# Youngju-Na/UFORecon

Hardware: AMD Instinct MI355X
Metric: rays/s (per-ray volume-rendering path, 64+64 hierarchical samples, DTU-shaped 3-view 512x640) (higher is better)
Workload: dtype f32; 1 GPU; configs[1]: full 512x640 frame = 327680 rays, 3 source views, 64+64 samples, rays sharded by row tiles over 1 GPU(s), depth/RGB tiles all-gathered; rays_per_frame=327680, chunk_rays=4096, side_streams=3

## Files before the change

uforecon_amd/csrc/api_weights_frame.hip:

```cpp
#include "api_common.h"
#include "ufr_layout_f16.h"

using namespace ufr;
using namespace ufr::api;

namespace {

int frame_check(const ufr_frame_desc* d) {
  UFR_REQUIRE(d, "frame desc is null");
  UFR_CHECK(check_views("frame desc", d->NV));
  UFR_REQUIRE(d->H >= 8 && d->W >= 8 && d->H % 4 == 0 && d->W % 4 == 0, "H,W must be multiples of 4 (got %dx%d)",
              d->H, d->W);
  UFR_REQUIRE(d->source_imgs && d->depth_info && d->feat, "null frame tensor");
  UFR_REQUIRE((long long)d->H * d->W < (1 << 24) && (long long)(d->H / 4) * (d->W / 4) * 32 * (d->NV - 1) < (1ll << 32),
              "image of %dx%d is too large for the gather's 24-bit texel indices", d->H, d->W);
  {
    const long long px = (long long)d->H * d->W, mpx = (long long)(d->H / 4) * (d->W / 4), lim = 1ll << 31;
    UFR_REQUIRE(px * 16 < lim && d->NV * mpx * 128 < lim && d->NV * mpx * 32 * (d->NV - 1) * 4 < lim,
                "frame of %dx%d with %d views: an image / feature-map buffer reaches 2 GiB (the gathers' zero-fill offset)",
                d->H, d->W, d->NV);
  }
  const bool has_vol = d->vol_feat[0] != nullptr;
  for (int s = 0; s < UFR_NUM_STAGES; ++s) {
    UFR_REQUIRE((d->vol_feat[s] != nullptr) == has_vol && (d->vol_weight[s] != nullptr) == has_vol,
                "volumes must be given for all stages or for none (stage %d)", s + 1);
    if (has_vol) UFR_REQUIRE(d->vol_D[s] >= 2 && d->vol_H[s] >= 2 && d->vol_W[s] >= 2, "degenerate volume (stage %d)", s + 1);
    if (has_vol)
      UFR_REQUIRE((long long)d->vol_D[s] * d->vol_H[s] < (1 << 24) && (long long)d->vol_W[s] * kVolCh < (1 << 24) &&
                      (long long)d->vol_D[s] * d->vol_H[s] * d->vol_W[s] * kVolCh * 4 < (1ll << 31),
                  "volume of stage %d is too large for the gather's 31-bit byte offsets (per view: < 2 GiB)", s + 1);
  }
  UFR_REQUIRE(d->source_poses && d->source_cam_pos && d->ref_cam_pos && d->w2c_row2, "null camera constants");
  return UFR_OK;
}

struct FrameWs { float *feat, *match, *rgb, *vol[UFR_NUM_STAGES]; unsigned* abs_max; };
FrameWs carve_frame(Carver& c, const ufr_frame_desc* d) {
  const size_t NV = d->NV, hw = (size_t)(d->H / 4) * (d->W / 4);
  FrameWs w = {};
  w.feat = c.f32(NV * hw * 32);
  if (d->match) w.match = c.f32(NV * hw * 32 * (NV - 1));
  w.rgb = c.f32(NV * d->H * d->W * 4);
  if (d->vol_feat[0])
    for (int s = 0; s < UFR_NUM_STAGES; ++s) w.vol[s] = c.f32(NV * d->vol_D[s] * d->vol_H[s] * d->vol_W[s] * kVolCh);
  w.abs_max = c.take<unsigned>(64);
  return w;
}

}

extern "C" {

size_t ufr_packed_weights_bytes(void) { return (size_t)blob_floats() * sizeof(float) + (size_t)kF16Bytes + (size_t)kBwdBytes + 16; }
size_t ufr_packed_bwd_halfwords(void) { return (size_t)kBwdHalfwords; }
size_t ufr_packed_fp32_floats(void) { return (size_t)blob_floats(); }
size_t ufr_packed_f16_halfwords(void) { return (size_t)kF16Halfwords; }
size_t ufr_packed_scale_table_offset(void) { return (size_t)scale_table_offset(); }
int ufr_packed_scale_table_entries(void) { return M_COUNT; }

int ufr_pack_plan_f16(int32_t* param_id, int32_t* elem, int32_t* plane) {
  UFR_REQUIRE(param_id && elem && plane, "ufr_pack_plan_f16: null output");
  for (int h = 0; h < kF16Halfwords; ++h) plan_entry_f16(h, &param_id[h], &elem[h], &plane[h]);
  return UFR_OK;
}

int ufr_pack_plan_bwd(int32_t* param_id, int32_t* elem, int32_t* plane) {
  UFR_REQUIRE(param_id && elem && plane, "ufr_pack_plan_bwd: null output");
  for (int h = 0; h < kBwdHalfwords; ++h) plan_entry_f16(kF16Halfwords + h, &param_id[h], &elem[h], &plane[h]);
  return UFR_OK;
}

int ufr_pack_plan(int32_t* param_id, int32_t* elem) {
  UFR_REQUIRE(param_id && elem, "ufr_pack_plan: null output");
  for (int i = 0; i < blob_floats(); ++i) {
    int p, e;
    plan_entry(i, &p, &e);
    param_id[i] = p;
    elem[i] = e;
  }
  return UFR_OK;
}

int ufr_weights_pack_for(const ufr_raw_weights* raw, void* packed, float input_abs_max, ufr_stream stream) {
  UFR_REQUIRE(raw && packed, "ufr_weights_pack: null argument");
  static_assert(sizeof(ufr_raw_weights) == sizeof(RawPtrs), "ufr_raw_weights must be P_COUNT pointers");
  RawPtrs rp;
  memcpy(&rp, raw, sizeof(rp));
  for (int i = 0; i < P_COUNT; ++i) UFR_REQUIRE(rp.p[i], "ufr_weights_pack: parameter %d is null", i);
  UFR_REQUIRE(input_abs_max > 0.f && input_abs_max <= 3.0e38f, "ufr_weights_pack_for: input_abs_max=%g must be positive and finite",
              (double)input_abs_max);
  hipStream_t s = static_cast<hipStream_t>(stream);
  UFR_STATUS_SLOT(sl);
  UFR_HIP(launch_pack_weights(rp, static_cast<float*>(packed), input_abs_max, status_word(sl), s));
  return status_leave(sl, s);
}

int ufr_weights_fit_frame(void* packed, const ufr_frame* frame, ufr_stream stream) {
  const FrameDev* f = frame_of(frame);
  UFR_REQUIRE(packed && f, "ufr_weights_fit_frame: null weights / frame handle not prepared");
  hipStream_t s = static_cast<hipStream_t>(stream);
  UFR_STATUS_SLOT(sl);
  UFR_HIP(launch_refit_weights(static_cast<float*>(packed), f->abs_max, status_word(sl), s));
  return UFR_OK;
}

int ufr_weights_pack(const ufr_raw_weights* raw, void* packed, ufr_stream stream) {
  return ufr_weights_pack_for(raw, packed, kDefaultInputAbsMax, stream);
}

size_t ufr_frame_workspace_bytes(const ufr_frame_desc* d) {
  if (frame_check(d) != UFR_OK) return 0;
  return carved_bytes(carve_frame, d);
}

int ufr_frame_prepare(const ufr_frame_desc* d, void* workspace, size_t workspace_bytes, ufr_frame* out,
                      ufr_stream stream) {
  UFR_CHECK(frame_check(d));
  UFR_REQUIRE(workspace && out, "ufr_frame_prepare: null workspace/out");
  Carver c(workspace);
  const FrameWs w = carve_frame(c, d);
  UFR_CHECK(check_workspace("ufr_frame_prepare", workspace_bytes, c.off));
  hipStream_t s = static_cast<hipStream_t>(stream);
  const int NV = d->NV, h = d->H / 4, hw = h * (d->W / 4);
  const bool has_vol = d->vol_feat[0] != nullptr;

  UFR_HIP(hipMemsetAsync(w.abs_max, 0, 256, s));
  UFR_HIP(launch_nchw_to_nhwc(d->feat, w.feat, NV, 32, hw, 32, s, w.abs_max));
  if (w.match) UFR_HIP(launch_nchw_to_nhwc(d->match, w.match, NV, 32 * (NV - 1), hw, 32 * (NV - 1), s));
  UFR_HIP(launch_nchw_to_nhwc(d->source_imgs, w.rgb, NV, 3, d->H * d->W, 4, s));
  if (has_vol)
    for (int st = 0; st < UFR_NUM_STAGES; ++st)
      UFR_HIP(launch_volume_pack(d->vol_feat[st], d->vol_weight[st], w.vol[st], NV, d->vol_D[st] * d->vol_H[st] * d->vol_W[st], s, w.abs_max));

  FrameDev f;
  memset(&f, 0, sizeof(f));
  f.NV = NV; f.H = d->H; f.W = d->W; f.h = h; f.w = d->W / 4; f.match_ch = 32 * (NV - 1);
  f.feat = w.feat; f.match = w.match; f.rgb = w.rgb; f.depth = d->depth_info;
  for (int st = 0; st < UFR_NUM_STAGES; ++st) {
    f.vol[st] = w.vol[st];
    if (has_vol) { f.vD[st] = d->vol_D[st]; f.vH[st] = d->vol_H[st]; f.vW[st] = d->vol_W[st]; }
  }
  for (int v = 0; v < NV; ++v) {
    memcpy(f.pose[v], d->source_poses + 16 * v, 12 * sizeof(float));
    memcpy(f.cam_pos[v], d->source_cam_pos + 3 * v, 3 * sizeof(float));
    memcpy(f.w2c_z[v], d->w2c_row2 + 4 * v, 4 * sizeof(float));
  }
  memcpy(f.ref_pos, d->ref_cam_pos, 3 * sizeof(float));
  f.vol_near = d->vol_near; f.vol_far = d->vol_far;
  f.abs_max = w.abs_max;
  f.magic = kFrameMagic;
  memset(out, 0, sizeof(*out));
  memcpy(out, &f, sizeof(f));
  return UFR_OK;
}

}
```

uforecon_amd/csrc/gather.hip:

```cpp
#include <algorithm>
#include <cstdlib>
#include "ufr_device.h"
#include "ufr_internal.h"
#include "volume_sample.h"

namespace ufr {

__device__ __forceinline__ f32x4 lerp_tap4_buf(__amdgpu_buffer_rsrc_t r, unsigned base, int stride_bytes, const Tap2& t, unsigned c4) {
  f32x4 v[4];
#pragma unroll
  for (int k = 0; k < 4; ++k)
    v[k] = buf_ld4(r, t.o[k] >= 0 ? base + __umul24((unsigned)t.o[k], (unsigned)stride_bytes) + c4 : kBufOut);
  f32x4 acc;
#pragma unroll
  for (int e = 0; e < 4; ++e) {
    float a = mul_rn(v[0][e], t.w[0]);
    a = fmaf(v[1][e], t.w[1], a);
    a = fmaf(v[2][e], t.w[2], a);
    acc[e] = fmaf(v[3][e], t.w[3], a);
  }
  return acc;
}

typedef int i32x4 __attribute__((ext_vector_type(4)));
// ... 162 lines not shown
    put_tap(sh_tapF + (v * 64 + p) * 8, taps_zeros(unnorm2d_nac(x, f.w), unnorm2d_nac(y, f.h), f.w, f.h));
    put_tap(sh_tapM + (v * 64 + p) * 8, taps_border(unnorm2d_ac(x, f.w), unnorm2d_ac(y, f.h), f.w, f.h));
    Tap2 tf = taps_zeros(unnorm2d_nac(x, f.W), unnorm2d_nac(y, f.H), f.W, f.H);
    const unsigned img_px = (unsigned)(f.H * f.W);
    f32x4 c4 = lerp_tap4_buf(buf_rsrc(f.rgb + (size_t)vu * img_px * 4, img_px * 16u), 0u, 16, tf, 0u);
    const float inb = (x <= 1.f && x >= -1.f && y <= 1.f && y >= -1.f) ? 1.f : 0.f;
    c4[3] = inb * mask_z;
    if (active) st4(rgb_out + ((size_t)pidx * NV + v) * 4, c4);
    float dv[4];
    const __amdgpu_buffer_rsrc_t rdepth = buf_rsrc(f.depth + (size_t)vu * img_px, img_px * 4u);
#pragma unroll
    for (int k = 0; k < 4; ++k) dv[k] = buf_ld1(rdepth, tf.o[k] >= 0 ? (unsigned)tf.o[k] * 4u : kBufOut);
    const float dm = fmaf(dv[3], tf.w[3], fmaf(dv[2], tf.w[2], fmaf(dv[1], tf.w[1], mul_rn(dv[0], tf.w[0]))));
    const float* R = f.w2c_z[v];
    float zc = fmaf(R[2], pz, fmaf(R[1], py, mul_rn(R[0], px))) + R[3];
    float delta = dm - zc;
    float pe[8];
#pragma unroll
    for (int k = 0; k < 4; ++k) {
      const float fr = 3.14159274101257324f * (float)(1 << k);
      pe[2 * k] = sinf(mul_rn(delta, fr));
      pe[2 * k + 1] = sinf(fmaf(delta, fr, 1.57079637050628662f));
    }
    if (active) {
      st4(xrow + pe_col, f32x4{pe[0], pe[1], pe[2], pe[3]});
      st4(xrow + pe_col + 4, f32x4{pe[4], pe[5], pe[6], pe[7]});
    }
    float ax = px - f.ref_pos[0], ay = py - f.ref_pos[1], az = pz - f.ref_pos[2];
    float bx = px - f.cam_pos[v][0], by = py - f.cam_pos[v][1], bz = pz - f.cam_pos[v][2];
    const float ra = __builtin_amdgcn_rcpf(sqrtf(ax * ax + ay * ay + az * az));
    const float rb = __builtin_amdgcn_rcpf(sqrtf(bx * bx + by * by + bz * bz));
    if (active) st4(dir_out + ((size_t)pidx * NV + v) * 4, f32x4{ax * ra - bx * rb, ay * ra - by * rb, az * ra - bz * rb, 0.f});
  }

  __syncthreads();
  UFR_G_PHASE(0)

  const int c8 = threadIdx.x & 7, grp = threadIdx.x >> 3;
  constexpr int n_grp = 64 * NV / 8;
  const unsigned map_px = (unsigned)(f.h * f.w);
  const __amdgpu_buffer_rsrc_t rfeat = buf_rsrc(f.feat, (unsigned)NV * map_px * 128u);
  const __amdgpu_buffer_rsrc_t rmatch = buf_rsrc(f.match, (unsigned)NV * map_px * (unsigned)f.match_ch * 4u);
  for (int item = grp; item < 64 * NV; item += n_grp) {
    const int iv = item >> 6, ip = item & 63;
    const int ipidx = point_of(ip);
    if (ipidx < P) {
      const Tap2 t = get_tap(sh_tapF + (iv * 64 + ip) * 8);
      st4(x_tokens + ((size_t)ipidx * NV + iv) * row_cols + 4 * c8,
          lerp_tap4_buf(rfeat, (unsigned)iv * map_px * 128u, 128, t, 16u * c8));
    }
  }
  if (!sim8_in)
  for (int item = grp; item < 64 * npair; item += n_grp) {
    const int q = item >> 6, ip = item & 63;
    int a = 0, rem = q;
    while (rem >= NV - 1 - a) { rem -= NV - 1 - a; ++a; }
    const int b = a + rem;
    const int va = a, ca = b, vb = b + 1, cb = a;
    const Tap2 ta = get_tap(sh_tapM + (va * 64 + ip) * 8), tb = get_tap(sh_tapM + (vb * 64 + ip) * 8);
    const unsigned mrow = (unsigned)f.match_ch * 4u;
    f32x4 fa = lerp_tap4_buf(rmatch, (unsigned)va * map_px * mrow + 128u * ca, (int)mrow, ta, 16u * c8);
    f32x4 fb = lerp_tap4_buf(rmatch, (unsigned)vb * map_px * mrow + 128u * cb, (int)mrow, tb, 16u * c8);
    float na = fmaxf(sqrtf(fa[0] * fa[0] + fa[1] * fa[1] + fa[2] * fa[2] + fa[3] * fa[3]), 1e-8f);
    float nb = fmaxf(sqrtf(fb[0] * fb[0] + fb[1] * fb[1] + fb[2] * fb[2] + fb[3] * fb[3]), 1e-8f);
    const float ra = __builtin_amdgcn_rcpf(na), rb = __builtin_amdgcn_rcpf(nb);
    sh_sim[(ip * npair + q) * 8 + c8] = (fa[0] * ra) * (fb[0] * rb) + (fa[1] * ra) * (fb[1] * rb) +
                                        (fa[2] * ra) * (fb[2] * rb) + (fa[3] * ra) * (fb[3] * rb);
  }
  __syncthreads();
  UFR_G_PHASE(1)

  float own[25];
  if (vol24_in) {
#pragma unroll
    for (int c = 0; c < 25; ++c) own[c] = 0.f;
  } else {
    const float zn = ((qz - f.vol_near) / (f.vol_far - f.vol_near)) * 2.f - 1.f;
    float fl[24], wl = 0.f;
#pragma unroll
    for (int s = 0; s < UFR_NUM_STAGES; ++s) {
      float fs[8], ws;
      const float* vol = f.vol[s];
      const unsigned vox = (unsigned)(f.vD[s] * f.vH[s] * f.vW[s]);
      sample_volume_buf(buf_rsrc(vol + (size_t)vu * vox * kVolCh, vox * (unsigned)(kVolCh * 4)), f.vD[s], f.vH[s], f.vW[s], x, y, zn,
                        fs, ws);
#pragma unroll
      for (int c = 0; c < 8; ++c) fl[8 * s + c] = fs[c];
      wl = s == 0 ? ws : wl + ws;
    }
#pragma unroll
    for (int c = 0; c < 24; ++c) own[c] = fl[c] * wl;
    own[24] = wl;
    if (v > 0) {
      float* dst = sh_vol + (p * (NV - 1) + (v - 1)) * 25;
#pragma unroll
      for (int c = 0; c < 25; ++c) dst[c] = own[c];
    }
  }
  __syncthreads();
  UFR_G_PHASE(2)

  if (v == 0) {
    float sim[8];
#pragma unroll
    for (int gi = 0; gi < 8; ++gi) {
      float s = 0.f;
      for (int q = 0; q < npair; ++q) s += sh_sim[(p * npair + q) * 8 + gi];
      sim[gi] = s / (float)npair;
      if (sim8_in) sim[gi] = sim8_in[(size_t)pc * 8 + gi];
    }
    {
      float Wsum = own[24];
      for (int n = 1; n < NV; ++n) Wsum += sh_vol[(p * (NV - 1) + n - 1) * 25 + 24];
      const float rW = 1.f / (Wsum + 1e-8f);
#pragma unroll
      for (int c = 0; c < 24; ++c) {
        float G = own[c];
        for (int n = 1; n < NV; ++n) G += sh_vol[(p * (NV - 1) + n - 1) * 25 + c];
        own[c] = G * rW;
        if (vol24_in) own[c] = vol24_in[(size_t)pc * 24 + c];
      }
    }
    __builtin_amdgcn_fence(__ATOMIC_RELEASE, "wavefront");
    __builtin_amdgcn_wave_barrier();
    __builtin_amdgcn_fence(__ATOMIC_ACQUIRE, "wavefront");
    float* mine = sh_sim + p * sim_slot;
    st4(mine, f32x4{sim[0], sim[1], sim[2], sim[3]});
    st4(mine + 4, f32x4{sim[4], sim[5], sim[6], sim[7]});
    float* ov = sh_out + p * out_stride;
#pragma unroll
    for (int c = 0; c < 24; c += 4) st4(ov + c, f32x4{own[c], own[c + 1], own[c + 2], own[c + 3]});
    UFR_G_PHASE(3)
    __builtin_amdgcn_fence(__ATOMIC_RELEASE, "wavefront");
    __builtin_amdgcn_wave_barrier();
    __builtin_amdgcn_fence(__ATOMIC_ACQUIRE, "wavefront");
    presim_block(ps, sh_sim, sim_slot, sh_out, out_stride, p);
  }
  __syncthreads();
  UFR_G_PHASE(4)

  int npts = P - pbase < 64 ? P - pbase : 64;
  if (SG) {
    const int nrays = (P - pbase + SN - 1) / SN;
    npts = nrays < kBlkRays ? kBlkSamples * nrays : 64;
  }
  const auto local_of = [=](int j) { return SG ? (int)((unsigned)j % kBlkSamples) * kBlkRays + (int)((unsigned)j / kBlkSamples) : j; };
  if (x_point) {
    for (int i = threadIdx.x; i < npts * 10; i += 64 * NV) {
      const int j = i / 10, c = i - j * 10, ip = local_of(j);
      st4(x_point + (size_t)point_of(ip) * kPointCols + 4 * c, ld4(sh_out + ip * out_stride + 4 * c));
    }
  } else {
    for (int i = threadIdx.x; i < npts * NV * 10; i += 64 * NV) {
      const int row = i / 10, c = i - row * 10, j = row / NV, ip = local_of(j);
      st4(x_tokens + ((size_t)point_of(ip) * NV + (row - j * NV)) * UFR_TOKEN_DIM + 32 + 4 * c, ld4(sh_out + ip * out_stride + 4 * c));
    }
  }
  if (vol24_out)
    for (int i = threadIdx.x; i < npts * 24; i += 64 * NV) {
      const int j = i / 24, ip = local_of(j);
      vol24_out[(size_t)point_of(ip) * 24 + (i - j * 24)] = sh_out[ip * out_stride + (i - j * 24)];
    }
  if (sim8_out)
    for (int i = threadIdx.x; i < npts * 8; i += 64 * NV) {
      const int ip = local_of(i >> 3);
      sim8_out[(size_t)point_of(ip) * 8 + (i & 7)] = sh_sim[ip * sim_slot + (i & 7)];
    }
  UFR_G_PHASE(5)
// ... 46 lines not shown
```

uforecon_amd/csrc/gather_bwd.hip:

```cpp
#include "ufr_internal.h"
#include "volume_sample.h"

namespace ufr {

constexpr int kGbwdRounds = 3;

template <int D, class T>
__device__ __forceinline__ T row_down(T v) {
  const int b = __builtin_bit_cast(int, v);
  return __builtin_bit_cast(T, __builtin_amdgcn_update_dpp(b, b, 0x100 + D, 0xf, 0xf, false));
}
template <int D, class T>
__device__ __forceinline__ T row_up(T v) {
  const int b = __builtin_bit_cast(int, v);
  return __builtin_bit_cast(T, __builtin_amdgcn_update_dpp(b, b, 0x110 + D, 0xf, 0xf, false));
}

struct VolGrads {
  float* rec[UFR_NUM_STAGES];
  unsigned char* touch[UFR_NUM_STAGES];
};
constexpr int kTouchGroup = 8;

__device__ __forceinline__ void scatter_records(float* __restrict__ base, unsigned char* __restrict__ touch, bool alive, int key,
                                                const float (&val)[9], float* slot, int lane) {
  const unsigned long long mask = __builtin_amdgcn_ballot_w64(alive);
  if (mask == 0ull) return;
  const int n = __builtin_popcountll(mask);
  const int rank = __builtin_popcountll(mask & ((1ull << lane) - 1ull));
  if (alive) {
    float* r = slot + rank * 10;
    r[0] = __builtin_bit_cast(float, key);
#pragma unroll
    for (int c = 0; c < 9; ++c) r[1 + c] = val[c];
  }
  __builtin_amdgcn_fence(__ATOMIC_RELEASE, "wavefront");
  __builtin_amdgcn_wave_barrier();
  __builtin_amdgcn_fence(__ATOMIC_ACQUIRE, "wavefront");
  const int sub = lane / 9, c = lane - 9 * sub;
  for (int r0 = 0; r0 < n; r0 += 7) {
    const int rec = r0 + sub;
    if (sub < 7 && rec < n) {
      const float* r = slot + rec * 10;
      const int k = __builtin_bit_cast(int, r[0]);
      unsafeAtomicAdd(base + (size_t)k * kVolCh + c, r[1 + c]);
      if (c == 0) touch[k / kTouchGroup] = 1;
    }
  }
  __builtin_amdgcn_fence(__ATOMIC_RELEASE, "wavefront");
  __builtin_amdgcn_wave_barrier();
  __builtin_amdgcn_fence(__ATOMIC_ACQUIRE, "wavefront");
}

__global__ void __launch_bounds__(448) gather_bwd_kernel(FrameDev f, VolGrads vg, const float* __restrict__ ray_o,
                                                          int o_stride, const float* __restrict__ ray_d,
                                                          const float* __restrict__ zval, const float* __restrict__ d_pv,
                                                          const int* __restrict__ pv_row,
                                                          int P, int SN) {
  extern __shared__ __attribute__((aligned(16))) float smem[];
  const int NV = f.NV;
  float* const rec_slot = smem + 64 * NV * 25 + (threadIdx.x >> 6) * 640;
  const int v = threadIdx.x >> 6, p = threadIdx.x & 63;
  const int pidx = blockIdx.x * 64 + p;
  const bool active = pidx < P;
  const int pc = active ? pidx : P - 1;
  const int ray = pc / SN;
  const float zz = zval[pc];
  const float* o = ray_o + (size_t)ray * o_stride;
  const float px = mul_add_unfused(zz, ray_d[3 * ray + 0], o[0]);
  const float py = mul_add_unfused(zz, ray_d[3 * ray + 1], o[1]);
  const float pz = mul_add_unfused(zz, ray_d[3 * ray + 2], o[2]);
  const float* M = f.pose[v];
  const float qx = fmaf(M[2], pz, fmaf(M[1], py, mul_rn(M[0], px))) + M[3];
  const float qy = fmaf(M[6], pz, fmaf(M[5], py, mul_rn(M[4], px))) + M[7];
  const float qz = fmaf(M[10], pz, fmaf(M[9], py, mul_rn(M[8], px))) + M[11];
  const float x = qx / qz, y = qy / qz;
  const float zn = ((qz - f.vol_near) / (f.vol_far - f.vol_near)) * 2.f - 1.f;

  float fl[24], wl = 0.f;
#pragma unroll
  for (int s = 0; s < UFR_NUM_STAGES; ++s) {
    float fs[8], ws;
    sample_volume(f.vol[s] + (size_t)v * f.vD[s] * f.vH[s] * f.vW[s] * kVolCh, f.vD[s], f.vH[s], f.vW[s], x, y, zn, fs, ws);
#pragma unroll
    for (int c = 0; c < 8; ++c) fl[8 * s + c] = fs[c];
    wl = s == 0 ? ws : wl + ws;
  }
  float* mine = smem + (p * NV + v) * 25;
#pragma unroll
  for (int c = 0; c < 24; ++c) mine[c] = fl[c] * wl;
  mine[24] = wl;
  __syncthreads();
  float Wsum = 0.f;
  for (int n = 0; n < NV; ++n) Wsum += smem[(p * NV + n) * 25 + 24];
  const float inv = 1.f / (Wsum + 1e-8f);
  const size_t pv_base = (size_t)(pv_row ? pv_row[pc] : pc) * 40;
  float dfl[24], dwl = 0.f;
#pragma unroll
  for (int c = 0; c < 24; ++c) {
    float G = 0.f;
    for (int n = 0; n < NV; ++n) G += smem[(p * NV + n) * 25 + c];
    const float dout = active ? d_pv[pv_base + c] : 0.f;
    dfl[c] = dout * wl * inv;
    dwl = fmaf(dout, (fl[c] - G * inv) * inv, dwl);
  }

#pragma unroll
  for (int s = 0; s < UFR_NUM_STAGES; ++s) {
    const int D = f.vD[s], H = f.vH[s], W = f.vW[s];
    const size_t plane = (size_t)D * H * W;
    float* grec = vg.rec[s] + (size_t)v * plane * kVolCh;
    unsigned char* gtouch = vg.touch[s] + (size_t)v * ((plane + kTouchGroup - 1) / kTouchGroup);
    const float ix = unnorm3d_ac(x, W), iy = unnorm3d_ac(y, H), iz = unnorm3d_ac(zn, D);
    const float fx = floorf(ix), fy = floorf(iy), fz = floorf(iz);
    const float wx[2] = {(fx + 1.f) - ix, ix - fx}, wy[2] = {(fy + 1.f) - iy, iy - fy}, wz[2] = {(fz + 1.f) - iz, iz - fz};
#pragma unroll
    for (int dy = 0; dy < 2; ++dy)
#pragma unroll
      for (int dx = 0; dx < 2; ++dx) {
        float val[2][9];
        int off[2];
        bool alive[2];
#pragma unroll
        for (int dz = 0; dz < 2; ++dz) {
          const float cx = fx + dx, cy = fy + dy, cz = fz + dz;
          const bool ok = active && cx >= 0.f && cx <= (float)(W - 1) && cy >= 0.f && cy <= (float)(H - 1) && cz >= 0.f &&
                          cz <= (float)(D - 1);
          const float wt = ok ? wx[dx] * wy[dy] * wz[dz] : 0.f;
          off[dz] = ok ? (((int)cz * H + (int)cy) * W + (int)cx) : -1 - (int)threadIdx.x - 1024 * dz;
#pragma unroll
          for (int c = 0; c < 8; ++c) val[dz][c] = wt * dfl[8 * s + c];
          val[dz][8] = wt * dwl;
          alive[dz] = ok;
        }
        {
          const int n_off0 = row_down<1>(off[0]);
          const int n_alive0 = row_down<1>((int)alive[0]);
          const bool give = alive[1] && n_alive0 && n_off0 == off[1] && (threadIdx.x & 15) != 15;
          const int p_give = row_up<1>((int)give);
#pragma unroll
          for (int c = 0; c < 9; ++c) {
            const float v_up = row_up<1>(val[1][c]);
            if (p_give && (threadIdx.x & 15) != 0) val[0][c] += v_up;
          }
          if (give) alive[1] = false;
        }
#pragma unroll
        for (int dz = 0; dz < 2; ++dz) {
          static_for<kGbwdRounds>([&](auto ri) __attribute__((always_inline)) {
            constexpr int d = 1 << decltype(ri)::value;
            const int k_dn = row_down<d>(off[dz]);
            const int k_up = row_up<d>(off[dz]);
            const int a_dn = row_down<d>((int)alive[dz]), a_up = row_up<d>((int)alive[dz]);
            const int pos = threadIdx.x & (2 * d - 1);
            const bool absorb = pos == 0 && alive[dz] && a_dn && k_dn == off[dz];
            const bool absorbed = pos == d && alive[dz] && a_up && k_up == off[dz];
#pragma unroll
            for (int c = 0; c < 9; ++c) {
              const float v_dn = row_down<d>(val[dz][c]);
              if (absorb) val[dz][c] += v_dn;
            }
            if (absorbed) alive[dz] = false;
          });
          scatter_records(grec, gtouch, alive[dz], off[dz], val[dz], rec_slot, threadIdx.x & 63);
        }
      }
  }
}

__global__ void __launch_bounds__(256) volume_unpack_kernel(float* __restrict__ rec, unsigned char* __restrict__ touch,
                                                             float* __restrict__ feat, float* __restrict__ weight, int S,
                                                             int accumulate) {
  const int s = blockIdx.x * blockDim.x + threadIdx.x, n = blockIdx.y;
  if (s >= S) return;
  const size_t groups = ((size_t)S + kTouchGroup - 1) / kTouchGroup;
  unsigned char* mark = touch + (size_t)n * groups + s / kTouchGroup;
  const bool touched = *mark != 0;
  float v[8], w = 0.f;
#pragma unroll
  for (int c = 0; c < 8; ++c) v[c] = 0.f;
  if (touched) {
    float* r = rec + ((size_t)n * S + s) * kVolCh;
    const f32x4 a = ld4(r), b = ld4(r + 4);
    w = r[8];
    v[0] = a[0]; v[1] = a[1]; v[2] = a[2]; v[3] = a[3];
    v[4] = b[0]; v[5] = b[1]; v[6] = b[2]; v[7] = b[3];
    st4(r, splat4(0.f));
    st4(r + 4, splat4(0.f));
    r[8] = 0.f;
    if (s % kTouchGroup == 0) *mark = 0;
  }
  float* fo = feat + (size_t)n * 8 * S + s;
  float* wo = weight + (size_t)n * S + s;
  if (accumulate) {
    if (touched) {
#pragma unroll
      for (int c = 0; c < 8; ++c) fo[(size_t)c * S] += v[c];
      *wo += w;
    }
  } else {
#pragma unroll
    for (int c = 0; c < 8; ++c) fo[(size_t)c * S] = v[c];
    *wo = w;
  }
}

static size_t touch_bytes(const FrameDev& f, int i) {
  const size_t groups = ((size_t)f.vD[i] * f.vH[i] * f.vW[i] + kTouchGroup - 1) / kTouchGroup;
  return (size_t)f.NV * groups;
}
size_t gather_bwd_scratch_floats(const FrameDev& f) {
  size_t n = 0, t = 0;
  for (int i = 0; i < UFR_NUM_STAGES; ++i) {
    n += (size_t)f.NV * f.vD[i] * f.vH[i] * f.vW[i] * kVolCh;
    t += (touch_bytes(f, i) + 15) / 16 * 16;
  }
  return n + t / 4;
}

hipError_t launch_gather_bwd(const FrameDev& f, float* const* grad_feat, float* const* grad_weight, const float* ray_o,
                             int o_stride, const float* ray_d, const float* z, const float* d_pv, const int* pv_row, int RN, int SN,
                             float* scratch, bool accumulate, bool scratch_zeroed, hipStream_t s) {
  const int P = RN * SN, NV = f.NV;
  if (!scratch_zeroed) {
    hipError_t e = hipMemsetAsync(scratch, 0, gather_bwd_scratch_floats(f) * sizeof(float), s);
    if (e != hipSuccess) return e;
  }
  VolGrads vg;
  size_t off = 0;
  for (int i = 0; i < UFR_NUM_STAGES; ++i) {
    vg.rec[i] = scratch + off;
    off += (size_t)NV * f.vD[i] * f.vH[i] * f.vW[i] * kVolCh;
  }
  unsigned char* tb = reinterpret_cast<unsigned char*>(scratch + off);
  for (int i = 0; i < UFR_NUM_STAGES; ++i) {
    vg.touch[i] = tb;
    tb += (touch_bytes(f, i) + 15) / 16 * 16;
  }
  const size_t lds = sizeof(float) * (64 * NV * 25 + NV * 640);
  hipLaunchKernelGGL(gather_bwd_kernel, dim3((P + 63) / 64), dim3(64 * NV), lds, s, f, vg, ray_o, o_stride, ray_d, z, d_pv, pv_row,
                     P, SN);
  for (int i = 0; i < UFR_NUM_STAGES; ++i) {
    const int S = f.vD[i] * f.vH[i] * f.vW[i];
    hipLaunchKernelGGL(volume_unpack_kernel, dim3((S + 255) / 256, NV), dim3(256), 0, s, vg.rec[i], vg.touch[i], grad_feat[i],
                       grad_weight[i], S, accumulate ? 1 : 0);
  }
  return hipGetLastError();
}

}
```

uforecon_amd/csrc/prep.hip:

```cpp
#include <cstdlib>
#include <mutex>

#include "ufr_internal.h"
#include "ufr_layout_f16.h"

namespace ufr {

__device__ __forceinline__ void wave_abs_max(float m, unsigned* __restrict__ abs_max) {
  unsigned b = __builtin_bit_cast(unsigned, m);
#pragma unroll
  for (int o = 32; o > 0; o >>= 1) b = max(b, (unsigned)__shfl_xor((int)b, o));
  if ((threadIdx.x & 63) == 0 && b > __atomic_load_n(abs_max, __ATOMIC_RELAXED)) atomicMax(abs_max, b);
}

template <int CPAD>
__global__ void __launch_bounds__(256) nchw_to_nhwc_kernel(const float* __restrict__ in, float* __restrict__ out,
                                                            int C, int S, unsigned* __restrict__ abs_max) {
  int s = blockIdx.x * blockDim.x + threadIdx.x;
  int n = blockIdx.y;
  float m = 0.f;
  if (s < S) {
    const float* src = in + (size_t)n * C * S + s;
    float v[CPAD];
#pragma unroll
    for (int c = 0; c < CPAD; ++c) v[c] = c < C ? src[(size_t)c * S] : 0.f;
    float4* dst = reinterpret_cast<float4*>(out + ((size_t)n * S + s) * CPAD);
#pragma unroll
    for (int c = 0; c < CPAD / 4; ++c) dst[c] = make_float4(v[4 * c], v[4 * c + 1], v[4 * c + 2], v[4 * c + 3]);
    if (abs_max) {
      unsigned mb = 0u;
#pragma unroll
      for (int c = 0; c < CPAD; ++c) mb = max(mb, __builtin_bit_cast(unsigned, v[c]) & 0x7fffffffu);
      m = __builtin_bit_cast(float, mb);
    }
  }
  if (abs_max) wave_abs_max(m, abs_max);
}

hipError_t launch_nchw_to_nhwc(const float* in, float* out, int N, int C, int S, int Cpad, hipStream_t s, unsigned* abs_max) {
  dim3 grid((S + 255) / 256, N), block(256);
  switch (Cpad) {
    case 4: hipLaunchKernelGGL(nchw_to_nhwc_kernel<4>, grid, block, 0, s, in, out, C, S, abs_max); break;
    case 32: hipLaunchKernelGGL(nchw_to_nhwc_kernel<32>, grid, block, 0, s, in, out, C, S, abs_max); break;
    case 64: hipLaunchKernelGGL(nchw_to_nhwc_kernel<64>, grid, block, 0, s, in, out, C, S, abs_max); break;
    case 96: hipLaunchKernelGGL(nchw_to_nhwc_kernel<96>, grid, block, 0, s, in, out, C, S, abs_max); break;
    case 128: hipLaunchKernelGGL(nchw_to_nhwc_kernel<128>, grid, block, 0, s, in, out, C, S, abs_max); break;
    case 160: hipLaunchKernelGGL(nchw_to_nhwc_kernel<160>, grid, block, 0, s, in, out, C, S, abs_max); break;
    case 192: hipLaunchKernelGGL(nchw_to_nhwc_kernel<192>, grid, block, 0, s, in, out, C, S, abs_max); break;
    default: return hipErrorInvalidValue;
  }
  return hipGetLastError();
}

__global__ void __launch_bounds__(256) volume_pack_kernel(const float* __restrict__ feat,
                                                           const float* __restrict__ weight,
                                                           float* __restrict__ out, int S, unsigned* __restrict__ abs_max) {
  int s = blockIdx.x * blockDim.x + threadIdx.x;
  int n = blockIdx.y;
  float m = 0.f;
  if (s < S) {
    const float* f = feat + (size_t)n * 8 * S + s;
    float v[8];
#pragma unroll
    for (int c = 0; c < 8; ++c) v[c] = f[(size_t)c * S];
    float w = weight[(size_t)n * S + s];
    float4* dst = reinterpret_cast<float4*>(out + ((size_t)n * S + s) * kVolCh);
    dst[0] = make_float4(v[0], v[1], v[2], v[3]);
    dst[1] = make_float4(v[4], v[5], v[6], v[7]);
    dst[2] = make_float4(w, 0.f, 0.f, 0.f);
    unsigned mb = 0u;
#pragma unroll
    for (int c = 0; c < 8; ++c) mb = max(mb, __builtin_bit_cast(unsigned, v[c]) & 0x7fffffffu);
    m = __builtin_bit_cast(float, mb);
  }
  if (abs_max) wave_abs_max(m, abs_max);
}

hipError_t launch_volume_pack(const float* feat, const float* weight, float* out, int N, int S, hipStream_t s, unsigned* abs_max) {
  dim3 grid((S + 255) / 256, N), block(256);
  hipLaunchKernelGGL(volume_pack_kernel, grid, block, 0, s, feat, weight, out, S, abs_max);
  return hipGetLastError();
}

__global__ void __launch_bounds__(256) vec_plan_kernel(int2* __restrict__ plan, int first, int n) {
  int i = first + blockIdx.x * blockDim.x + threadIdx.x;
  if (i >= n) return;
  int p, e;
  plan_entry(i, &p, &e);
  plan[i - first] = make_int2(p, e);
}
__global__ void __launch_bounds__(256) pack_weights_kernel(RawPtrs raw, const int2* __restrict__ plan, float* __restrict__ packed,
                                                            int first, int n) {
  int i = first + blockIdx.x * blockDim.x + threadIdx.x;
  if (i >= n) return;
  const int2 src = plan[i - first];
  packed[i] = src.x >= 0 ? raw.p[src.x][src.y] : 0.f;
}

namespace {
__device__ int plane_exponent(float bound, int lo, int hi) {
  int e;
  const float f = frexpf(bound, &e);
  return max(lo, min(hi, f == 0.5f ? 16 - e : 15 - e));
}
}

constexpr int kStatVecs = 18;
__device__ constexpr int kStatVecParam[kStatVecs][2] = {{P_VT_N1W, 80}, {P_VT_N1B, 80}, {P_VT_N2W, 80}, {P_VT_N2B, 80}, {P_RT_N1W, 88},
                                                        {P_RT_N1B, 88}, {P_RT_N2W, 88}, {P_RT_N2B, 88}, {P_DM_B0, 32}, {P_DM_B2, 16},
                                                        {P_DM_B4, 1}, {P_RW_B0, 16}, {P_RW_B2, 8}, {P_RW_B4, 1}, {P_VIEW_TOKEN, 80},
                                                        {P_PS_B0, 32}, {P_PS_B2, 32}, {P_PS_B4, 16}};
constexpr int kStatMats = M_COUNT + 3;
__device__ inline void stat_mat(int b, int* param, int* k_raw, int* out_dim) {
  if (b < M_COUNT) {
    const MatDesc d = mat_desc(b);
    *param = d.param; *k_raw = d.k_raw; *out_dim = d.out_dim;
  } else {
    *param = b == M_COUNT ? P_PS_W0 : b == M_COUNT + 1 ? P_PS_W2 : P_PS_W4;
    *k_raw = b == M_COUNT ? 8 : 32;
    *out_dim = b == M_COUNT + 2 ? 16 : 32;
  }
}
static_assert(2 * kStatMats + kStatVecs <= kStatBoundSlot && kStatBoundSlot < kStatFloats, "the statistics region of the scale table (ufr_layout.h)");
constexpr int kStatThreads = 1024;
__global__ void __launch_bounds__(kStatThreads) weight_stats_kernel(RawPtrs raw, float* __restrict__ stats, int* __restrict__ flag) {
  __shared__ float red[3][kStatThreads / 64];
  __shared__ float rowsum[176];
  __shared__ float part[8 * kStatThreads];
  const int b = blockIdx.x, wave = threadIdx.x >> 6, lane = threadIdx.x & 63;
  float m = 0.f, rs = 0.f;
  bool nf = false;
  if (b < kStatMats) {
    struct { int param, k_raw, out_dim; } d;
    stat_mat(b, &d.param, &d.k_raw, &d.out_dim);
    const float4* w4 = reinterpret_cast<const float4*>(raw.p[d.param]);
    for (int r = threadIdx.x; r < d.out_dim; r += kStatThreads) rowsum[r] = 0.f;
    __syncthreads();
    const int n4 = d.out_dim * d.k_raw / 4;
    const bool quads = d.k_raw % 4 == 0;
    float4 v[8];
#pragma unroll
    for (int u = 0; u < 8; ++u) {
      const int i4 = threadIdx.x + u * kStatThreads;
      v[u] = w4[i4 < n4 ? i4 : n4 - 1];
    }
#pragma unroll
    for (int u = 0; u < 8; ++u) {
      const int i4 = threadIdx.x + u * kStatThreads;
      const bool in = i4 < n4;
      const float e[4] = {in ? fabsf(v[u].x) : 0.f, in ? fabsf(v[u].y) : 0.f, in ? fabsf(v[u].z) : 0.f, in ? fabsf(v[u].w) : 0.f};
      const float s4 = (e[0] + e[1]) + (e[2] + e[3]);
      nf |= !(s4 <= 3.0e38f);
      m = fmaxf(fmaxf(m, fmaxf(e[0], e[1])), fmaxf(e[2], e[3]));
      if (quads) {
        if (i4 < n4) part[i4] = s4;
        continue;
      }
      const int r0 = (4 * i4) / d.k_raw, r3 = (4 * i4 + 3) / d.k_raw;
      const bool one_row = i4 < n4 && r0 == r3 && r0 == __shfl(r0, 0);
      if (__builtin_amdgcn_ballot_w64(one_row) == ~0ull) {
        float t = s4;
        for (int o = 32; o > 0; o >>= 1) t += __shfl_xor(t, o);
        if (lane == 0) atomicAdd(&rowsum[r0], t);
// ... 227 lines not shown
```

uforecon_amd/csrc/ufr_internal.h:

```cpp
#pragma once
#include <hip/hip_runtime.h>
#include <stdint.h>

#include <mutex>

#include "../../include/ufr.h"
#include "ufr_layout.h"

namespace ufr {

constexpr int kVolCh = 12;

struct FrameDev {
  int32_t NV, H, W, h, w, match_ch;
  const float* feat;
  const float* match;
  const float* rgb;
  const float* depth;
  const float* vol[UFR_NUM_STAGES];
  int32_t vD[UFR_NUM_STAGES], vH[UFR_NUM_STAGES], vW[UFR_NUM_STAGES];
  float pose[UFR_MAX_VIEWS][12];
  float cam_pos[UFR_MAX_VIEWS][3];
  float w2c_z[UFR_MAX_VIEWS][4];
  float ref_pos[3];
  float vol_near, vol_far;
  uint32_t magic;
  const unsigned* abs_max;
};
static_assert(sizeof(FrameDev) <= sizeof(ufr_frame), "ufr_frame too small");
constexpr uint32_t kFrameMagic = 0x55465246u;

struct PreSim {
  const float *w0, *b0, *w2, *b2, *w4, *b4;
};

struct LdsAttrOnce {
  std::once_flag flag[16];
  hipError_t err[16];
  hipError_t set(const void* kernel, int bytes) {
    int dev = 0;
    if (hipGetDevice(&dev) != hipSuccess || dev < 0 || dev >= 16) return hipErrorInvalidDevice;
    std::call_once(flag[dev], [&] { err[dev] = hipFuncSetAttribute(kernel, hipFuncAttributeMaxDynamicSharedMemorySize, bytes); });
    return err[dev];
  }
};

hipError_t launch_nchw_to_nhwc(const float* in, float* out, int N, int C, int S, int Cpad, hipStream_t s, unsigned* abs_max = nullptr);
hipError_t launch_volume_pack(const float* feat, const float* weight, float* out, int N, int S, hipStream_t s, unsigned* abs_max = nullptr);
hipError_t launch_ray_setup(const int64_t* ray_idx, const float* ray_d, const float* cam_ray_d, int HW, float near_z,
                            float far_z, int RN, float* rd_out, float* near_out, float* far_out, float* camz_out,
                            const float* ray_o_host, float* ray_o_out, hipStream_t s);
hipError_t launch_sample_fixed(const float* near, const float* far, const float* U, int u_stride, float* z, int RN,
                               int SN, hipStream_t s);
hipError_t launch_importance_merge(const float* weight, const float* z, const float* U2, int u_stride, float* z_fine,
                                   float* z_all, int RN, int SN, int PN, float* z_new, int* src_row, hipStream_t s);
hipError_t launch_order_pe(float* table, int SN, hipStream_t s);
hipError_t launch_points(const float* ray_o, int o_stride, const float* ray_d, const float* z, float* pts, int RN,
                         int SN, hipStream_t s);
constexpr int kViewCols = 40, kPointCols = 40;
hipError_t launch_gather(const FrameDev& f, const PreSim& ps, const float* ray_o, int o_stride, const float* ray_d,
                         const float* z, int RN, int SN, float* x_tokens, float* x_point, float* rgb, float* dir, float* sim8,
                         float* vol24, float* xy, float* mask_z, const float* vol24_in, const float* sim8_in,
                         hipStream_t s);
hipError_t launch_view_transformer(const float* packed, const float* x_tokens, const float* x_point, const float* rgb,
                                   const float* dir, int P, int NV, float* token0, float* radiance, float* view_out, bool lowp, int* status,
                                   hipStream_t s);
hipError_t launch_ray_transformer(const float* packed, const float* token0, const int* tok_row, const float* order_pe,
                                  int RN, int SN, float* srdf, float* ray_out, bool lowp, int* status, hipStream_t s);
hipError_t launch_composite(const float* z, const float* radiance, const int* rad_row, const float* srdf,
                            const float* variance, int RN, int SN, float* rgb, float* depth, float* opacity, float* weight,
                            const float* camz, float* depth_z, hipStream_t s);
hipError_t launch_render_loss(const float* rgb_c, const float* depth_c, const float* rgb_f, const float* depth_f,
                              const float* rgb_gt, const float* depth_gt, const float* near_far, int nf_stride, int B, int RN,
                              float weight_rgb, float weight_depth, float* loss, float* d_rgb_c, float* d_depth_c,
                              float* d_rgb_f, float* d_depth_f, hipStream_t s);
hipError_t launch_composite_bwd(const float* z, const float* radiance, const int* rad_row, bool accumulate, const float* srdf,
                                const float* variance, int RN, int SN, const float* d_rgb, const float* d_depth,
                                const float* d_opacity, const float* d_weight, float* d_radiance, float* d_srdf,
                                float* d_variance, hipStream_t s);
struct GradPtrs { float* p[P_COUNT]; };
__device__ __forceinline__ void atomic_add_f32(float* p, float v) { unsafeAtomicAdd(p, v); }
int view_tape_blocks(int P, int NV);
hipError_t launch_view_tape(const float* packed, const float* x_tokens, const float* rgb, const float* dir, int P, int NV,
                            float* token0, float* radiance, float* tape, bool lowp, int* status, hipStream_t s);
hipError_t launch_view_dgrad(const float* packed, const float* tape, const float* rgbm, const float* d_tok_a,
                             const float* d_tok_b, const float* d_radiance, int P, int NV, float* dbuf, float* d_pv,
                             const GradPtrs& gp, bool lowp, hipStream_t s);
hipError_t launch_view_wgrad(const float* tape, const float* dbuf, int n_blocks, const GradPtrs& gp, bool lowp, hipStream_t s);
hipError_t launch_ray_tape(const float* packed, const float* token0, const int* tok_row, const float* order_pe, int RN, int SN,
                           float* srdf, float* tape, float* ray_state, bool lowp, int* status, hipStream_t s);
hipError_t launch_ray_dgrad(const float* packed, const float* tape, const float* ray_state, const float* d_srdf, const int* tok_row,
                            bool accumulate, int RN, int SN, float* dbuf, float* d_tok_a, float* d_tok_b, const GradPtrs& gp, bool lowp,
                            hipStream_t s);
hipError_t launch_ray_wgrad(const float* tape, const float* dbuf, int n_blocks, const GradPtrs& gp, bool lowp, hipStream_t s);
hipError_t launch_presim_bwd(const RawPtrs& wp, const GradPtrs& gp, const float* sim8, const float* d_pv, int P, bool lowp,
                             hipStream_t s);
size_t gather_bwd_scratch_floats(const FrameDev& f);
hipError_t launch_gather_bwd(const FrameDev& f, float* const* grad_feat, float* const* grad_weight, const float* ray_o,
                             int o_stride, const float* ray_d, const float* z, const float* d_pv, const int* pv_row, int RN,
                             int SN, float* scratch, bool accumulate, bool scratch_zeroed, hipStream_t s);
struct FmtWeights {
  const float *wq, *bq, *wk, *bk, *wv, *bv, *wo, *bo, *w1, *b1, *w2, *b2, *n1w, *n1b, *n2w, *n2b;
};
int fmt_state_parts(int S);
hipError_t launch_fmt_layer(const FmtWeights& w, const float* x, const float* src, int N, int T, int S, float* out,
                            float* state, hipStream_t s);
hipError_t launch_pack_weights(const RawPtrs& raw, float* packed, float input_abs_max, int* range_flag, hipStream_t s);
hipError_t launch_refit_weights(float* packed, const unsigned* frame_bound, int* range_flag, hipStream_t s);
hipError_t launch_tsdf_integrate(float* tsdf, float* weight, float* color, const int* dim, const float* origin,
                                 float voxel_size, float trunc_margin, const float* K, const float* P,
                                 const float* depth_im, const float* color_im, int im_h, int im_w, float obs_weight,
                                 int integrate_color, hipStream_t s);
int mcubes_tiles(const int* dim);
hipError_t launch_mcubes_count(const float* vol, const int* dim, float level, int* tile_counts, hipStream_t s);
hipError_t launch_mcubes_scan(const int* tile_counts, int n_tiles, long long* tile_off, long long* totals, hipStream_t s);
hipError_t launch_mcubes_verts(const float* vol, const int* dim, float level, const long long* tile_off, int* index,
                               float* verts, float* normals, long long n_verts, hipStream_t s);
hipError_t launch_mcubes_faces(const float* vol, const int* dim, float level, const long long* tile_off, const int* index,
                               int* faces, long long n_faces, hipStream_t s);
hipError_t launch_similarity_field(const FrameDev& f, const float* gx, const float* gy, const float* gz, const int* dim, float* u,
                                   unsigned char* n_vis, int min_views, hipStream_t s);
long long chamfer_blocks(long long n);
hipError_t launch_points_cell_keys(const double* pts, long long n, const double* origin, double cell, long long* keys,
                                   hipStream_t s);
hipError_t launch_mesh_sample_count(const double* verts, const int* faces, long long V, long long F, double density,
                                    long long* tri_off, long long* block_tot, hipStream_t s);
hipError_t launch_mesh_sample_scan(const long long* block_tot, long long n_blocks, long long* block_off, long long* total,
                                   hipStream_t s);
hipError_t launch_mesh_sample_emit(const double* verts, const int* faces, long long V, long long F, double density,
                                   const long long* tri_off, const long long* block_off, double* out, long long capacity,
                                   hipStream_t s);
// ... 113 lines not shown
```

uforecon_amd/csrc/volume_sample.h:

```cpp
#pragma once
#include "ufr_device.h"
#include "ufr_internal.h"

namespace ufr {

__device__ __forceinline__ void sample_volume(const float* __restrict__ vol, int D, int H, int W, float x, float y,
                                              float zn, float (&f)[8], float& wgt) {
  float ix = unnorm3d_ac(x, W), iy = unnorm3d_ac(y, H), iz = unnorm3d_ac(zn, D);
  float fx = floorf(ix), fy = floorf(iy), fz = floorf(iz);
  float wx[2] = {(fx + 1.f) - ix, ix - fx}, wy[2] = {(fy + 1.f) - iy, iy - fy}, wz[2] = {(fz + 1.f) - iz, iz - fz};
  f32x4 a0 = splat4(0.f), a1 = splat4(0.f);
  float aw = 0.f;
#pragma unroll
  for (int dz = 0; dz < 2; ++dz)
#pragma unroll
    for (int dy = 0; dy < 2; ++dy)
#pragma unroll
      for (int dx = 0; dx < 2; ++dx) {
        float cx = fx + dx, cy = fy + dy, cz = fz + dz;
        bool ok = cx >= 0.f && cx <= (float)(W - 1) && cy >= 0.f && cy <= (float)(H - 1) && cz >= 0.f &&
                  cz <= (float)(D - 1);
        if (ok) {
          const float wt = mul_rn(mul_rn(wx[dx], wy[dy]), wz[dz]);
          const unsigned row = __umul24((unsigned)(int)cz, (unsigned)H) + (unsigned)(int)cy;
          const float* t = vol + (__umul24(row, (unsigned)(W * kVolCh)) + __umul24((unsigned)(int)cx, (unsigned)kVolCh));
          const f32x4 v0 = ld4(t), v1 = ld4(t + 4);
#pragma unroll
          for (int e = 0; e < 4; ++e) {
            a0[e] = mul_add_unfused(v0[e], wt, a0[e]);
            a1[e] = mul_add_unfused(v1[e], wt, a1[e]);
          }
          aw = mul_add_unfused(t[8], wt, aw);
        }
      }
  f[0] = a0[0]; f[1] = a0[1]; f[2] = a0[2]; f[3] = a0[3];
  f[4] = a1[0]; f[5] = a1[1]; f[6] = a1[2]; f[7] = a1[3];
  wgt = aw;
}

__device__ __forceinline__ void sample_volume_buf(__amdgpu_buffer_rsrc_t r, int D, int H, int W, float x, float y, float zn,
                                                  float (&f)[8], float& wgt) {
  float ix = unnorm3d_ac(x, W), iy = unnorm3d_ac(y, H), iz = unnorm3d_ac(zn, D);
  float fx = floorf(ix), fy = floorf(iy), fz = floorf(iz);
  float wx[2] = {(fx + 1.f) - ix, ix - fx}, wy[2] = {(fy + 1.f) - iy, iy - fy}, wz[2] = {(fz + 1.f) - iz, iz - fz};
  unsigned off[8];
  float wt[8];
#pragma unroll
  for (int dz = 0; dz < 2; ++dz)
#pragma unroll
    for (int dy = 0; dy < 2; ++dy)
#pragma unroll
      for (int dx = 0; dx < 2; ++dx) {
        const int k = 4 * dz + 2 * dy + dx;
        float cx = fx + dx, cy = fy + dy, cz = fz + dz;
        bool ok = cx >= 0.f && cx <= (float)(W - 1) && cy >= 0.f && cy <= (float)(H - 1) && cz >= 0.f &&
                  cz <= (float)(D - 1);
        wt[k] = mul_rn(mul_rn(wx[dx], wy[dy]), wz[dz]);
        const unsigned row = __umul24((unsigned)(int)cz, (unsigned)H) + (unsigned)(int)cy;
        const unsigned texel = __umul24(row, (unsigned)W) + (unsigned)(int)cx;
        off[k] = ok ? texel * (unsigned)(kVolCh * 4) : kBufOut;
      }
  f32x4 v0[8], v1[8];
  float v2[8];
#pragma unroll
  for (int k = 0; k < 8; ++k) {
    v0[k] = buf_ld4(r, off[k]);
    v1[k] = buf_ld4(r, off[k] + 16u);
    v2[k] = buf_ld1(r, off[k] + 32u);
  }
  f32x4 a0 = splat4(0.f), a1 = splat4(0.f);
  float aw = 0.f;
#pragma unroll
  for (int k = 0; k < 8; ++k) {
#pragma unroll
    for (int e = 0; e < 4; ++e) {
      a0[e] = mul_add_unfused(v0[k][e], wt[k], a0[e]);
      a1[e] = mul_add_unfused(v1[k][e], wt[k], a1[e]);
    }
    aw = mul_add_unfused(v2[k], wt[k], aw);
  }
  f[0] = a0[0]; f[1] = a0[1]; f[2] = a0[2]; f[3] = a0[3];
  f[4] = a1[0]; f[5] = a1[1]; f[6] = a1[2]; f[7] = a1[3];
  wgt = aw;
}

}
```

Before: 2.795 million rays/s.

## Split volume weight channel out of packed 12-float texels into separate plane

Volume texels shrink from a padded 12-float record (8 features + weight + 3 pad) to 8 floats. The weight channel is now read from the caller's original weight tensor through a second buffer resource. The aim is less memory footprint and fewer wasted bytes per trilinear gather, with 32-byte aligned texels. In exchange each corner issues a load to a separate array, losing the locality of having the weight next to its features. The backward gradient scratch keeps the 12-wide stride.

```diff
diff --git a/uforecon_amd/csrc/api_weights_frame.hip b/uforecon_amd/csrc/api_weights_frame.hip
--- a/uforecon_amd/csrc/api_weights_frame.hip
+++ b/uforecon_amd/csrc/api_weights_frame.hip
@@ -24,11 +24,13 @@
   for (int s = 0; s < UFR_NUM_STAGES; ++s) {
     UFR_REQUIRE((d->vol_feat[s] != nullptr) == has_vol && (d->vol_weight[s] != nullptr) == has_vol,
                 "volumes must be given for all stages or for none (stage %d)", s + 1);
-    if (has_vol) UFR_REQUIRE(d->vol_D[s] >= 2 && d->vol_H[s] >= 2 && d->vol_W[s] >= 2, "degenerate volume (stage %d)", s + 1);
-    if (has_vol)
-      UFR_REQUIRE((long long)d->vol_D[s] * d->vol_H[s] < (1 << 24) && (long long)d->vol_W[s] * kVolCh < (1 << 24) &&
-                      (long long)d->vol_D[s] * d->vol_H[s] * d->vol_W[s] * kVolCh * 4 < (1ll << 31),
-                  "volume of stage %d is too large for the gather's 31-bit byte offsets (per view: < 2 GiB)", s + 1);
+    if (has_vol) UFR_REQUIRE(d->vol_D[s] >= 1 && d->vol_H[s] >= 2 && d->vol_W[s] >= 2, "degenerate volume (stage %d)", s + 1);
+    if (has_vol) {
+      const long long vox = (long long)d->vol_D[s] * d->vol_H[s] * d->vol_W[s];
+      UFR_REQUIRE((long long)d->vol_D[s] * d->vol_H[s] < (1 << 24) && d->vol_W[s] < (1 << 24) &&
+                      vox * kVolCh * 4 < (1ll << 31) && vox * 4 < (1ll << 31),
+                  "volume of stage %d is too large for the gather's 31-bit byte offsets (per view: < 2 GiB of features)", s + 1);
+    }
   }
   UFR_REQUIRE(d->source_poses && d->source_cam_pos && d->ref_cam_pos && d->w2c_row2, "null camera constants");
   return UFR_OK;
@@ -130,7 +132,7 @@
   UFR_HIP(launch_nchw_to_nhwc(d->source_imgs, w.rgb, NV, 3, d->H * d->W, 4, s));
   if (has_vol)
     for (int st = 0; st < UFR_NUM_STAGES; ++st)
-      UFR_HIP(launch_volume_pack(d->vol_feat[st], d->vol_weight[st], w.vol[st], NV, d->vol_D[st] * d->vol_H[st] * d->vol_W[st], s, w.abs_max));
+      UFR_HIP(launch_volume_pack(d->vol_feat[st], w.vol[st], NV, d->vol_D[st] * d->vol_H[st] * d->vol_W[st], s, w.abs_max));
 
   FrameDev f;
   memset(&f, 0, sizeof(f));
@@ -138,6 +140,7 @@
   f.feat = w.feat; f.match = w.match; f.rgb = w.rgb; f.depth = d->depth_info;
   for (int st = 0; st < UFR_NUM_STAGES; ++st) {
     f.vol[st] = w.vol[st];
+    f.vol_w[st] = has_vol ? d->vol_weight[st] : nullptr;
     if (has_vol) { f.vD[st] = d->vol_D[st]; f.vH[st] = d->vol_H[st]; f.vW[st] = d->vol_W[st]; }
   }
   for (int v = 0; v < NV; ++v) {
diff --git a/uforecon_amd/csrc/gather.hip b/uforecon_amd/csrc/gather.hip
--- a/uforecon_amd/csrc/gather.hip
+++ b/uforecon_amd/csrc/gather.hip
@@ -268,8 +268,8 @@
       float fs[8], ws;
       const float* vol = f.vol[s];
       const unsigned vox = (unsigned)(f.vD[s] * f.vH[s] * f.vW[s]);
-      sample_volume_buf(buf_rsrc(vol + (size_t)vu * vox * kVolCh, vox * (unsigned)(kVolCh * 4)), f.vD[s], f.vH[s], f.vW[s], x, y, zn,
-                        fs, ws);
+      sample_volume_buf(buf_rsrc(vol + (size_t)vu * vox * kVolCh, vox * (unsigned)(kVolCh * 4)),
+                        buf_rsrc(f.vol_w[s] + (size_t)vu * vox, vox * 4u), f.vD[s], f.vH[s], f.vW[s], x, y, zn, fs, ws);
 #pragma unroll
       for (int c = 0; c < 8; ++c) fl[8 * s + c] = fs[c];
       wl = s == 0 ? ws : wl + ws;
diff --git a/uforecon_amd/csrc/gather_bwd.hip b/uforecon_amd/csrc/gather_bwd.hip
--- a/uforecon_amd/csrc/gather_bwd.hip
+++ b/uforecon_amd/csrc/gather_bwd.hip
@@ -3,6 +3,7 @@
 
 namespace ufr {
 
+constexpr int kGradCh = 12;
 constexpr int kGbwdRounds = 3;
 
 template <int D, class T>
@@ -43,7 +44,7 @@
     if (sub < 7 && rec < n) {
       const float* r = slot + rec * 10;
       const int k = __builtin_bit_cast(int, r[0]);
-      unsafeAtomicAdd(base + (size_t)k * kVolCh + c, r[1 + c]);
+      unsafeAtomicAdd(base + (size_t)k * kGradCh + c, r[1 + c]);
       if (c == 0) touch[k / kTouchGroup] = 1;
     }
   }
@@ -81,7 +82,8 @@
 #pragma unroll
   for (int s = 0; s < UFR_NUM_STAGES; ++s) {
     float fs[8], ws;
-    sample_volume(f.vol[s] + (size_t)v * f.vD[s] * f.vH[s] * f.vW[s] * kVolCh, f.vD[s], f.vH[s], f.vW[s], x, y, zn, fs, ws);
+    const size_t vox = (size_t)v * f.vD[s] * f.vH[s] * f.vW[s];
+    sample_volume(f.vol[s] + vox * kVolCh, f.vol_w[s] + vox, f.vD[s], f.vH[s], f.vW[s], x, y, zn, fs, ws);
 #pragma unroll
     for (int c = 0; c < 8; ++c) fl[8 * s + c] = fs[c];
     wl = s == 0 ? ws : wl + ws;
@@ -109,7 +111,7 @@
   for (int s = 0; s < UFR_NUM_STAGES; ++s) {
     const int D = f.vD[s], H = f.vH[s], W = f.vW[s];
     const size_t plane = (size_t)D * H * W;
-    float* grec = vg.rec[s] + (size_t)v * plane * kVolCh;
+    float* grec = vg.rec[s] + (size_t)v * plane * kGradCh;
     unsigned char* gtouch = vg.touch[s] + (size_t)v * ((plane + kTouchGroup - 1) / kTouchGroup);
     const float ix = unnorm3d_ac(x, W), iy = unnorm3d_ac(y, H), iz = unnorm3d_ac(zn, D);
     const float fx = floorf(ix), fy = floorf(iy), fz = floorf(iz);
@@ -180,7 +182,7 @@
 #pragma unroll
   for (int c = 0; c < 8; ++c) v[c] = 0.f;
   if (touched) {
-    float* r = rec + ((size_t)n * S + s) * kVolCh;
+    float* r = rec + ((size_t)n * S + s) * kGradCh;
     const f32x4 a = ld4(r), b = ld4(r + 4);
     w = r[8];
     v[0] = a[0]; v[1] = a[1]; v[2] = a[2]; v[3] = a[3];
@@ -212,7 +214,7 @@
 size_t gather_bwd_scratch_floats(const FrameDev& f) {
   size_t n = 0, t = 0;
   for (int i = 0; i < UFR_NUM_STAGES; ++i) {
-    n += (size_t)f.NV * f.vD[i] * f.vH[i] * f.vW[i] * kVolCh;
+    n += (size_t)f.NV * f.vD[i] * f.vH[i] * f.vW[i] * kGradCh;
     t += (touch_bytes(f, i) + 15) / 16 * 16;
   }
   return n + t / 4;
@@ -230,7 +232,7 @@
   size_t off = 0;
   for (int i = 0; i < UFR_NUM_STAGES; ++i) {
     vg.rec[i] = scratch + off;
-    off += (size_t)NV * f.vD[i] * f.vH[i] * f.vW[i] * kVolCh;
+    off += (size_t)NV * f.vD[i] * f.vH[i] * f.vW[i] * kGradCh;
   }
   unsigned char* tb = reinterpret_cast<unsigned char*>(scratch + off);
   for (int i = 0; i < UFR_NUM_STAGES; ++i) {
diff --git a/uforecon_amd/csrc/prep.hip b/uforecon_amd/csrc/prep.hip
--- a/uforecon_amd/csrc/prep.hip
+++ b/uforecon_amd/csrc/prep.hip
@@ -52,9 +52,8 @@
   return hipGetLastError();
 }
 
-__global__ void __launch_bounds__(256) volume_pack_kernel(const float* __restrict__ feat,
-                                                           const float* __restrict__ weight,
-                                                           float* __restrict__ out, int S, unsigned* __restrict__ abs_max) {
+__global__ void __launch_bounds__(256) volume_pack_kernel(const float* __restrict__ feat, float* __restrict__ out, int S,
+                                                           unsigned* __restrict__ abs_max) {
   int s = blockIdx.x * blockDim.x + threadIdx.x;
   int n = blockIdx.y;
   float m = 0.f;
@@ -63,11 +62,9 @@
     float v[8];
 #pragma unroll
     for (int c = 0; c < 8; ++c) v[c] = f[(size_t)c * S];
-    float w = weight[(size_t)n * S + s];
     float4* dst = reinterpret_cast<float4*>(out + ((size_t)n * S + s) * kVolCh);
     dst[0] = make_float4(v[0], v[1], v[2], v[3]);
     dst[1] = make_float4(v[4], v[5], v[6], v[7]);
-    dst[2] = make_float4(w, 0.f, 0.f, 0.f);
     unsigned mb = 0u;
 #pragma unroll
     for (int c = 0; c < 8; ++c) mb = max(mb, __builtin_bit_cast(unsigned, v[c]) & 0x7fffffffu);
@@ -76,9 +73,9 @@
   if (abs_max) wave_abs_max(m, abs_max);
 }
 
-hipError_t launch_volume_pack(const float* feat, const float* weight, float* out, int N, int S, hipStream_t s, unsigned* abs_max) {
+hipError_t launch_volume_pack(const float* feat, float* out, int N, int S, hipStream_t s, unsigned* abs_max) {
   dim3 grid((S + 255) / 256, N), block(256);
-  hipLaunchKernelGGL(volume_pack_kernel, grid, block, 0, s, feat, weight, out, S, abs_max);
+  hipLaunchKernelGGL(volume_pack_kernel, grid, block, 0, s, feat, out, S, abs_max);
   return hipGetLastError();
 }
 
diff --git a/uforecon_amd/csrc/ufr_internal.h b/uforecon_amd/csrc/ufr_internal.h
--- a/uforecon_amd/csrc/ufr_internal.h
+++ b/uforecon_amd/csrc/ufr_internal.h
@@ -9,7 +9,7 @@
 
 namespace ufr {
 
-constexpr int kVolCh = 12;
+constexpr int kVolCh = 8;
 
 struct FrameDev {
   int32_t NV, H, W, h, w, match_ch;
@@ -18,6 +18,7 @@
   const float* rgb;
   const float* depth;
   const float* vol[UFR_NUM_STAGES];
+  const float* vol_w[UFR_NUM_STAGES];
   int32_t vD[UFR_NUM_STAGES], vH[UFR_NUM_STAGES], vW[UFR_NUM_STAGES];
   float pose[UFR_MAX_VIEWS][12];
   float cam_pos[UFR_MAX_VIEWS][3];
@@ -46,7 +47,7 @@
 };
 
 hipError_t launch_nchw_to_nhwc(const float* in, float* out, int N, int C, int S, int Cpad, hipStream_t s, unsigned* abs_max = nullptr);
-hipError_t launch_volume_pack(const float* feat, const float* weight, float* out, int N, int S, hipStream_t s, unsigned* abs_max = nullptr);
+hipError_t launch_volume_pack(const float* feat, float* out, int N, int S, hipStream_t s, unsigned* abs_max = nullptr);
 hipError_t launch_ray_setup(const int64_t* ray_idx, const float* ray_d, const float* cam_ray_d, int HW, float near_z,
                             float far_z, int RN, float* rd_out, float* near_out, float* far_out, float* camz_out,
                             const float* ray_o_host, float* ray_o_out, hipStream_t s);
diff --git a/uforecon_amd/csrc/volume_sample.h b/uforecon_amd/csrc/volume_sample.h
--- a/uforecon_amd/csrc/volume_sample.h
+++ b/uforecon_amd/csrc/volume_sample.h
@@ -4,8 +4,8 @@
 
 namespace ufr {
 
-__device__ __forceinline__ void sample_volume(const float* __restrict__ vol, int D, int H, int W, float x, float y,
-                                              float zn, float (&f)[8], float& wgt) {
+__device__ __forceinline__ void sample_volume(const float* __restrict__ vol, const float* __restrict__ wvol, int D, int H, int W,
+                                              float x, float y, float zn, float (&f)[8], float& wgt) {
   float ix = unnorm3d_ac(x, W), iy = unnorm3d_ac(y, H), iz = unnorm3d_ac(zn, D);
   float fx = floorf(ix), fy = floorf(iy), fz = floorf(iz);
   float wx[2] = {(fx + 1.f) - ix, ix - fx}, wy[2] = {(fy + 1.f) - iy, iy - fy}, wz[2] = {(fz + 1.f) - iz, iz - fz};
@@ -23,14 +23,15 @@
         if (ok) {
           const float wt = mul_rn(mul_rn(wx[dx], wy[dy]), wz[dz]);
           const unsigned row = __umul24((unsigned)(int)cz, (unsigned)H) + (unsigned)(int)cy;
-          const float* t = vol + (__umul24(row, (unsigned)(W * kVolCh)) + __umul24((unsigned)(int)cx, (unsigned)kVolCh));
+          const unsigned texel = __umul24(row, (unsigned)W) + (unsigned)(int)cx;
+          const float* t = vol + texel * (unsigned)kVolCh;
           const f32x4 v0 = ld4(t), v1 = ld4(t + 4);
 #pragma unroll
           for (int e = 0; e < 4; ++e) {
             a0[e] = mul_add_unfused(v0[e], wt, a0[e]);
             a1[e] = mul_add_unfused(v1[e], wt, a1[e]);
           }
-          aw = mul_add_unfused(t[8], wt, aw);
+          aw = mul_add_unfused(wvol[texel], wt, aw);
         }
       }
   f[0] = a0[0]; f[1] = a0[1]; f[2] = a0[2]; f[3] = a0[3];
@@ -38,12 +39,12 @@
   wgt = aw;
 }
 
-__device__ __forceinline__ void sample_volume_buf(__amdgpu_buffer_rsrc_t r, int D, int H, int W, float x, float y, float zn,
-                                                  float (&f)[8], float& wgt) {
+__device__ __forceinline__ void sample_volume_buf(__amdgpu_buffer_rsrc_t r, __amdgpu_buffer_rsrc_t rw, int D, int H, int W, float x,
+                                                  float y, float zn, float (&f)[8], float& wgt) {
   float ix = unnorm3d_ac(x, W), iy = unnorm3d_ac(y, H), iz = unnorm3d_ac(zn, D);
   float fx = floorf(ix), fy = floorf(iy), fz = floorf(iz);
   float wx[2] = {(fx + 1.f) - ix, ix - fx}, wy[2] = {(fy + 1.f) - iy, iy - fy}, wz[2] = {(fz + 1.f) - iz, iz - fz};
-  unsigned off[8];
+  unsigned off[8], offw[8];
   float wt[8];
 #pragma unroll
   for (int dz = 0; dz < 2; ++dz)
@@ -59,6 +60,7 @@
         const unsigned row = __umul24((unsigned)(int)cz, (unsigned)H) + (unsigned)(int)cy;
         const unsigned texel = __umul24(row, (unsigned)W) + (unsigned)(int)cx;
         off[k] = ok ? texel * (unsigned)(kVolCh * 4) : kBufOut;
+        offw[k] = ok ? texel * 4u : kBufOut;
       }
   f32x4 v0[8], v1[8];
   float v2[8];
@@ -66,7 +68,7 @@
   for (int k = 0; k < 8; ++k) {
     v0[k] = buf_ld4(r, off[k]);
     v1[k] = buf_ld4(r, off[k] + 16u);
-    v2[k] = buf_ld1(r, off[k] + 32u);
+    v2[k] = buf_ld1(rw, offw[k]);
   }
   f32x4 a0 = splat4(0.f), a1 = splat4(0.f);
   float aw = 0.f;
```

After: 2.800 million rays/s (median of 4 runs). Within noise of the previous version (+0.2%).
